# KTH-RPL/HiMo

Hardware: AMD Instinct MI355X
Metric: lidar_frames_per_sec_120k (higher is better)
Workload: dtype f16x2 (two-term split fp16, x = h + l with exact subnormals, on the matrix cores; float32 accumulate; ~22-bit products); 1 GPU; per-frame pipeline: pillarise 3 sweeps (512x512 grid) -> SeFlow++-style encoder/decoder + GRU head (random-init, self-specified: reference network source absent) -> per-point flow -> ego-motion removal + dt0 + flow2compDis -> comp_dis; points_per_frame=120000, sweeps_per_frame=3, parallelism=frames sharded x1, refined_output=False, batches_in_flight=3, matrix_arithmetic=f16x2, samples_per_backbone_launch=16, collectives=none (single process)

## Files before the change

himo_amd/csrc/conv.hip:

```cpp
#include "conv_plan.h"

namespace himo {

template <int KS, int S, int BN, int EPI, int MI>
__global__ __launch_bounds__(256) void conv_mfma_kernel(ConvArgs a) {
    constexpr int BM = 64 * MI, BK = 16, TH = 4 * MI, TW = 16;
    constexpr int PH = KS == 1 ? 1 : (TH - 1) * S + KS;
    constexpr int PW = KS == 1 ? BM : (TW - 1) * S + KS;
    constexpr int PP = PH * PW + 1;
    constexpr int WN = BN / 2, NI = WN / 32;
    constexpr int T = KS * KS;
    constexpr bool kPatchDouble = S == 1;
    constexpr int kPatchBufs = kPatchDouble ? 2 : 1;
    constexpr int kPatchItems = PH * PW * (BK / 4);
    constexpr int kPatchPerThread = (kPatchItems + 255) / 256;
    constexpr int kWPerThread = BK * (BN / 4) / 256;
    constexpr int kPatchFloats = kPatchBufs * BK * PP, kWFloats = 2 * BK * BN;
    static_assert(kPatchFloats % 4 == 0, "weight slabs stay 16-byte aligned");
    __shared__ __attribute__((aligned(16))) float smem[kPatchFloats + kWFloats < 4096 ? 4096 : kPatchFloats + kWFloats];
    auto& patchT = *reinterpret_cast<float (*)[kPatchBufs][BK * PP]>(smem);
    auto& wt = *reinterpret_cast<float (*)[2][BK * BN]>(smem + kPatchFloats);

    const int n_tiles_n = (a.Cout + BN - 1) / BN;
    int bid = xcd_block_id(blockIdx.x, gridDim.x);
// ... 261 lines not shown
    const unsigned item = blockIdx.x * 256u + threadIdx.x;
    const unsigned ox = item / cq, q = item - ox * cq;
    if (ox >= 2u * (unsigned)a.W) return;
    const int oy = (int)blockIdx.y;
    const float sy = a.ry * (float)oy, sx = a.rx * (float)ox;
    const int y0 = (int)sy, x0 = (int)sx;
    const int y1 = y0 + (y0 < a.H - 1 ? 1 : 0), x1 = x0 + (x0 < a.W - 1 ? 1 : 0);
    const float ly1 = sy - (float)y0, lx1 = sx - (float)x0;
    const float ly0 = 1.f - ly1, lx0 = 1.f - lx1;
    const float* row0 = a.x + (int64_t)y0 * a.W * a.x_pitch + q * 8;
    const float* row1 = a.x + (int64_t)y1 * a.W * a.x_pitch + q * 8;
    const unsigned c0 = (unsigned)x0 * (unsigned)a.x_pitch, c1 = (unsigned)x1 * (unsigned)a.x_pitch;
    float o[8];
#pragma unroll
    for (int part = 0; part < 2; ++part) {
        const float4 v00 = *reinterpret_cast<const float4*>(row0 + c0 + part * 4), v01 = *reinterpret_cast<const float4*>(row0 + c1 + part * 4);
        const float4 v10 = *reinterpret_cast<const float4*>(row1 + c0 + part * 4), v11 = *reinterpret_cast<const float4*>(row1 + c1 + part * 4);
        o[part * 4 + 0] = ly0 * (lx0 * v00.x + lx1 * v01.x) + ly1 * (lx0 * v10.x + lx1 * v11.x);
        o[part * 4 + 1] = ly0 * (lx0 * v00.y + lx1 * v01.y) + ly1 * (lx0 * v10.y + lx1 * v11.y);
        o[part * 4 + 2] = ly0 * (lx0 * v00.z + lx1 * v01.z) + ly1 * (lx0 * v10.z + lx1 * v11.z);
        o[part * 4 + 3] = ly0 * (lx0 * v00.w + lx1 * v01.w) + ly1 * (lx0 * v10.w + lx1 * v11.w);
    }
    unsigned h[8], l[8];
#pragma unroll
    for (int k = 0; k < 8; ++k) split2_rounded(o[k], h[k], l[k]);
    unsigned char* rec = reinterpret_cast<unsigned char*>(a.y + ((int64_t)oy * (2 * a.W) + ox) * a.y_pitch + (q >> 1) * 16) + (q & 1) * 16;
    *reinterpret_cast<uint4*>(rec) = make_uint4(h[0] | (h[1] << 16), h[2] | (h[3] << 16), h[4] | (h[5] << 16), h[6] | (h[7] << 16));
    *reinterpret_cast<uint4*>(rec + 32) = make_uint4(l[0] | (l[1] << 16), l[2] | (l[3] << 16), l[4] | (l[5] << 16), l[6] | (l[7] << 16));
}

constexpr int kUpRows = 8;
template <int CQ>
__global__ __launch_bounds__(256) void upsample2x_split_lds_kernel(UpArgs a) {
    constexpr int PX = 256 / CQ, NC = PX / 2 + 2, NR = kUpRows / 2 + 2, C = CQ * 8, C4 = C / 4;
    constexpr int CP = C + 4;
    __shared__ __attribute__((aligned(16))) float tile[NR * NC * CP];
    a.x += (int64_t)blockIdx.z * a.x_bs;
    a.y += (int64_t)blockIdx.z * a.y_bs;
    const int ox0 = (int)blockIdx.x * PX, oy0 = (int)blockIdx.y * kUpRows;
    const int cy0 = (int)(a.ry * (float)oy0), cx0 = (int)(a.rx * (float)ox0);
    for (int e = threadIdx.x; e < NR * NC * C4; e += 256) {
        const int px = e / C4, j = e - px * C4;
        const int r = px / NC, c = px - r * NC;
        const int yy = min(cy0 + r, a.H - 1), xx = min(cx0 + c, a.W - 1);
        *reinterpret_cast<float4*>(&tile[px * CP + j * 4]) = *reinterpret_cast<const float4*>(a.x + ((int64_t)yy * a.W + xx) * a.x_pitch + j * 4);
    }
    __syncthreads();
    const int q = threadIdx.x % CQ, p = threadIdx.x / CQ;
    const int ox = ox0 + p;
    if (ox >= 2 * a.W) return;
    const float sx = a.rx * (float)ox;
    const int x0 = (int)sx;
    const int x1 = x0 + (x0 < a.W - 1 ? 1 : 0);
    const float lx1 = sx - (float)x0, lx0 = 1.f - lx1;
    const int t0 = (x0 - cx0) * CP + q * 8, t1 = (x1 - cx0) * CP + q * 8;
#pragma unroll
    for (int r = 0; r < kUpRows; ++r) {
        const int oy = oy0 + r;
        if (oy >= 2 * a.H) break;
        const float sy = a.ry * (float)oy;
        const int y0 = (int)sy;
        const int y1 = y0 + (y0 < a.H - 1 ? 1 : 0);
        const float ly1 = sy - (float)y0, ly0 = 1.f - ly1;
        const float* r0 = &tile[(y0 - cy0) * NC * CP], * r1 = &tile[(y1 - cy0) * NC * CP];
        float o[8];
#pragma unroll
        for (int part = 0; part < 2; ++part) {
            const float4 v00 = *reinterpret_cast<const float4*>(r0 + t0 + part * 4), v01 = *reinterpret_cast<const float4*>(r0 + t1 + part * 4);
            const float4 v10 = *reinterpret_cast<const float4*>(r1 + t0 + part * 4), v11 = *reinterpret_cast<const float4*>(r1 + t1 + part * 4);
            o[part * 4 + 0] = ly0 * (lx0 * v00.x + lx1 * v01.x) + ly1 * (lx0 * v10.x + lx1 * v11.x);
            o[part * 4 + 1] = ly0 * (lx0 * v00.y + lx1 * v01.y) + ly1 * (lx0 * v10.y + lx1 * v11.y);
            o[part * 4 + 2] = ly0 * (lx0 * v00.z + lx1 * v01.z) + ly1 * (lx0 * v10.z + lx1 * v11.z);
            o[part * 4 + 3] = ly0 * (lx0 * v00.w + lx1 * v01.w) + ly1 * (lx0 * v10.w + lx1 * v11.w);
        }
        unsigned h[8], l[8];
#pragma unroll
        for (int k = 0; k < 8; ++k) split2_rounded(o[k], h[k], l[k]);
        unsigned char* rec = reinterpret_cast<unsigned char*>(a.y + ((int64_t)oy * (2 * a.W) + ox) * a.y_pitch + (q >> 1) * 16) + (q & 1) * 16;
        *reinterpret_cast<uint4*>(rec) = make_uint4(h[0] | (h[1] << 16), h[2] | (h[3] << 16), h[4] | (h[5] << 16), h[6] | (h[7] << 16));
        *reinterpret_cast<uint4*>(rec + 32) = make_uint4(l[0] | (l[1] << 16), l[2] | (l[3] << 16), l[4] | (l[5] << 16), l[6] | (l[7] << 16));
    }
}

template <int KS, int S, int BN, int MI>
static void launch_epi(const ConvPlan& p, hipStream_t s) {
    switch (p.epi) {
        case kEpiBias: hipLaunchKernelGGL((conv_mfma_kernel<KS, S, BN, kEpiBias, MI>), p.grid, dim3(256), 0, s, p.args); break;
        case kEpiBiasBnGelu: hipLaunchKernelGGL((conv_mfma_kernel<KS, S, BN, kEpiBiasBnGelu, MI>), p.grid, dim3(256), 0, s, p.args); break;
        case kEpiBiasGelu: hipLaunchKernelGGL((conv_mfma_kernel<KS, S, BN, kEpiBiasGelu, MI>), p.grid, dim3(256), 0, s, p.args); break;
        case kEpiGruZR: hipLaunchKernelGGL((conv_mfma_kernel<KS, S, BN, kEpiGruZR, MI>), p.grid, dim3(256), 0, s, p.args); break;
        case kEpiBiasRelu: hipLaunchKernelGGL((conv_mfma_kernel<KS, S, BN, kEpiBiasRelu, MI>), p.grid, dim3(256), 0, s, p.args); break;
        case kEpiReluMask: hipLaunchKernelGGL((conv_mfma_kernel<KS, S, BN, kEpiReluMask, MI>), p.grid, dim3(256), 0, s, p.args); break;
        default: hipLaunchKernelGGL((conv_mfma_kernel<KS, S, BN, kEpiGruQ, MI>), p.grid, dim3(256), 0, s, p.args); break;
    }
}

template <int KS, int S>
static void launch_tile(const ConvPlan& p, hipStream_t s) {
    if (p.bn == 128) { if (p.mi == 2) launch_epi<KS, S, 128, 2>(p, s); else launch_epi<KS, S, 128, 1>(p, s); }
    else { if (p.mi == 2) launch_epi<KS, S, 64, 2>(p, s); else launch_epi<KS, S, 64, 1>(p, s); }
}

void launch_conv_f32(const ConvPlan& p, hipStream_t s) {
    if (p.ks == 1) launch_tile<1, 1>(p, s);
    else if (p.stride == 1) launch_tile<3, 1>(p, s);
    else launch_tile<3, 2>(p, s);
}

}

using namespace himo;

extern "C" int himo_conv2d(const himo_conv_desc* d, void* stream) {
    if (!d) return HIMO_ERR_INVALID_ARGUMENT;
    ConvPlan p;
    const int st = plan_conv(*d, p);
    if (st != HIMO_OK) return st;
    hipStream_t s = (hipStream_t)stream;
    {
        ProfScope ps(p.prof_name, s);
        switch (p.family) {
            case kConvF32: launch_conv_f32(p, s); break;
            case kConvStaged: launch_conv_staged(p, s); break;
            case kConvFromL2: launch_conv_from_l2(p, s); break;
            case kConvPresplit3: launch_conv_presplit3(p, s); break;
            case kConvPresplit1: launch_conv_presplit1(p, s); break;
        }
    }
    HIMO_LAUNCH_CHECK(p.prof_name);
    return HIMO_OK;
}

extern "C" int himo_upsample2x(const float* d_x, int x_pitch, int h, int w, int c, float* d_y, int y_pitch, void* stream) {
    return himo_upsample2x_batch(1, d_x, 0, x_pitch, h, w, c, d_y, 0, y_pitch, stream);
}

extern "C" int himo_upsample2x_batch(int n, const float* d_x, int64_t x_batch_stride, int x_pitch, int h, int w, int c, float* d_y,
                                     int64_t y_batch_stride, int y_pitch, void* stream) {
    return himo_upsample2x_batch_ex(n, d_x, x_batch_stride, x_pitch, h, w, c, d_y, y_batch_stride, y_pitch, 0, stream);
}

extern "C" int himo_upsample2x_batch_ex(int n, const float* d_x, int64_t x_batch_stride, int x_pitch, int h, int w, int c, float* d_y,
                                        int64_t y_batch_stride, int y_pitch, int out_split, void* stream) {
    if (out_split && ((c & 15) || (y_pitch & 15) || (y_batch_stride & 15) || (reinterpret_cast<uintptr_t>(d_y) & 63))) return HIMO_ERR_INVALID_ARGUMENT;
    if (n < 1 || !d_x || !d_y || h < 1 || w < 1 || c < 4 || (c & 3) || (x_pitch & 3) || (y_pitch & 3) || (x_batch_stride & 3) ||
        (y_batch_stride & 3))
        return HIMO_ERR_INVALID_ARGUMENT;
    UpArgs a{};
    a.x = d_x; a.x_pitch = x_pitch; a.H = h; a.W = w; a.C = c; a.y = d_y; a.y_pitch = y_pitch;
    a.x_bs = x_batch_stride; a.y_bs = y_batch_stride; a.out_split = out_split ? 1 : 0;
    a.ry = h > 1 ? (float)(h - 1) / (float)(2 * h - 1) : 0.f;
    a.rx = w > 1 ? (float)(w - 1) / (float)(2 * w - 1) : 0.f;
    ProfScope ps("upsample2x_kernel", (hipStream_t)stream);
    if (out_split && (c == 64 || c == 128 || c == 256) && (2 * h + kUpRows - 1) / kUpRows <= 65535 && n <= 65535) {
        const int cq = c / 8, px = 256 / cq;
        const dim3 grid((2 * w + px - 1) / px, (2 * h + kUpRows - 1) / kUpRows, n);
        if (cq == 8) hipLaunchKernelGGL(upsample2x_split_lds_kernel<8>, grid, dim3(256), 0, (hipStream_t)stream, a);
        else if (cq == 16) hipLaunchKernelGGL(upsample2x_split_lds_kernel<16>, grid, dim3(256), 0, (hipStream_t)stream, a);
        else hipLaunchKernelGGL(upsample2x_split_lds_kernel<32>, grid, dim3(256), 0, (hipStream_t)stream, a);
        HIMO_LAUNCH_CHECK("upsample2x_split_lds_kernel");
        return HIMO_OK;
    }
    if (out_split && 2 * h <= 65535 && n <= 65535 && (int64_t)w * x_pitch < ((int64_t)1 << 31)) {
        const unsigned row_items = (unsigned)(2 * w) * (unsigned)(c / 8);
        hipLaunchKernelGGL(upsample2x_split_row_kernel, dim3((row_items + 255) / 256, 2 * h, n), dim3(256), 0, (hipStream_t)stream, a);
        HIMO_LAUNCH_CHECK("upsample2x_split_row_kernel");
        return HIMO_OK;
    }
    const int64_t total = (int64_t)(2 * h) * (2 * w) * (c / (out_split ? 8 : 4));
    const dim3 grid((unsigned)((total + 255) / 256), n);
    if (out_split) hipLaunchKernelGGL(upsample2x_kernel<true>, grid, dim3(256), 0, (hipStream_t)stream, a);
    else hipLaunchKernelGGL(upsample2x_kernel<false>, grid, dim3(256), 0, (hipStream_t)stream, a);
    HIMO_LAUNCH_CHECK("upsample2x_kernel");
    return HIMO_OK;
}
```

himo_amd/csrc/conv_plan.h:

```cpp
#pragma once
#include "conv_common.h"

namespace himo {

enum ConvFamily {
    kConvF32,
    kConvStaged,
    kConvFromL2,
    kConvPresplit3,
    kConvPresplit1
};

struct ConvPlan {
    ConvFamily family;
    ConvArgs args;
    int ks, stride, epi, fmt;
    int bn, mi, ph, nt;
    const void* w_packed;
    dim3 grid;
    const char* prof_name;
};

void launch_conv_f32(const ConvPlan& p, hipStream_t s);
void launch_conv_staged(const ConvPlan& p, hipStream_t s);
void launch_conv_from_l2(const ConvPlan& p, hipStream_t s);
void launch_conv_presplit3(const ConvPlan& p, hipStream_t s);
void launch_conv_presplit1(const ConvPlan& p, hipStream_t s);

inline int64_t blocks_for(const ConvArgs& a, int th, int tw, int bn) {
    const int64_t tiles = th ? (int64_t)((a.Ho + th - 1) / th) * ((a.Wo + tw - 1) / tw) : ((int64_t)a.Ho * a.Wo + tw - 1) / tw;
    return (int64_t)a.N * tiles * ((a.Cout + bn - 1) / bn);
}

inline bool below_2gb(int64_t pixels, int pitch) { return pixels * pitch * 4 < ((int64_t)1 << 31); }

inline const char* conv_prof_name(int ks, int stride, int fmt) {
    static const char* const names[3][4] = {
        {"conv1x1_mfma_kernel", "conv1x1_bf16x3_kernel", "conv1x1_f16x2_kernel", "conv1x1_bf16x2_kernel"},
        {"conv3x3_mfma_kernel", "conv3x3_bf16x3_kernel", "conv3x3_f16x2_kernel", "conv3x3_bf16x2_kernel"},
        {"conv3x3s2_mfma_kernel", "conv3x3s2_bf16x3_kernel", "conv3x3s2_f16x2_kernel", "conv3x3s2_bf16x2_kernel"}};
    return names[ks == 1 ? 0 : stride == 2 ? 2 : 1][fmt < 0 ? 0 : fmt == 1 ? 2 : fmt == 2 ? 3 : 1];
}

inline void plan_staged_tile(ConvPlan& p, int rows_per_mi, int tw, bool keep128, int hint) {
    const ConvArgs& a = p.args;
    auto blocks = [&](int bn, int mi) { return p.ks == 1 ? blocks_for(a, 0, 64 * mi, bn) : blocks_for(a, rows_per_mi * mi, tw, bn); };
    const bool can128 = a.Cout >= 128 && (a.Cout % 128) == 0;
    int bn = can128 ? 128 : 64, mi = 2;
    if (blocks(bn, mi) < 512) mi = 1;
    if (blocks(bn, mi) < 512 && bn == 128 && !keep128) bn = 64;
    const int hb = hint >> 4, hm = hint & 15;
    if ((hb == 64 || (hb == 128 && can128)) && (hm == 1 || hm == 2)) { bn = hb; mi = hm; }
    p.bn = bn; p.mi = mi;
    p.grid = dim3((unsigned)blocks(bn, mi));
}

inline void plan_rows_tile(ConvPlan& p, int ph, int mi, int nt) {
    p.ph = ph; p.mi = mi; p.nt = nt; p.bn = (4 / ph) * 32 * nt;
    p.grid = dim3((unsigned)(p.ks == 1 ? blocks_for(p.args, 0, mi * ph * 32, p.bn) : blocks_for(p.args, mi * ph, 32, p.bn)));
}

inline bool plan_from_l2(ConvPlan& p, int rows_hint) {
    ConvArgs& a = p.args;
    const bool vec = vec_store_ok(a);
    if (p.epi == kEpiGruZR || p.epi == kEpiGruQ) return false;
    if (p.fmt == 2 && (p.epi != kEpiBias || (a.act_flags & ~(kActAccumulate | kActStuffedIn)))) return false;
    if ((a.act_flags & kActAccumulate) && (p.fmt != 2 || !vec)) return false;
    if ((a.act_flags & kActStuffedIn) && (p.fmt != 2 || p.stride != 1)) return false;
    if (!below_2gb((int64_t)a.H * a.W, a.x_pitch)) return false;
    const bool ph_ok = p.stride == 1 && p.fmt != 0;
    const int ph_hint = (ph_ok && (rows_hint == 5 || rows_hint == 6)) ? 2 : (ph_ok && (rows_hint == 9 || rows_hint == 10)) ? 4 : 0;
    if (!ph_hint && rows_hint > 4) return false;
    const bool wide = a.Cout > 64 && ph_hint == 0;
    const int ph = ph_hint ? ph_hint : (wide ? 1 : 2);
    int mi = blocks_for(a, 4 * ph, 32, (4 / ph) * 32) >= 1024 ? 4 : 2;
    if (rows_hint == 4 || rows_hint == 2 || rows_hint == 1) mi = rows_hint;
    if (ph_hint) mi = rows_hint & 3;
    if (p.stride == 2) mi = (rows_hint == 1 || rows_hint == 2) ? rows_hint : (wide ? 2 : 1);
    p.family = kConvFromL2;
    plan_rows_tile(p, ph, mi, 1);
    p.prof_name = conv_prof_name(3, p.stride, p.fmt);
    if (vec && (!(a.act_flags & kActSplitOut) || !(a.Cout & 15))) a.act_flags |= kActVecStore;
    return true;
}

inline int plan_presplit(ConvPlan& p, int rows_hint) {
    ConvArgs& a = p.args;
    if (!below_2gb((int64_t)a.H * a.W, a.x_pitch)) return HIMO_ERR_UNSUPPORTED;
    if (a.act_flags & kActRowMask) {
        p.family = kConvPresplit3;
        p.prof_name = "conv3x3_masked_f16x2_kernel";
        plan_rows_tile(p, 4, 2, 2);
        return HIMO_OK;
    }
    const bool wide = a.Cout > 64, vec = vec_store_ok(a), pinned = rows_hint == 4 || rows_hint == 2 || rows_hint == 1;
    const int ph = wide ? 1 : 2;
    p.family = p.ks == 1 ? kConvPresplit1 : kConvPresplit3;
    p.prof_name = conv_prof_name(p.ks, p.stride, 1);
    if (vec) a.act_flags |= kActVecStore;
    if (p.ks == 1) {
        int mi = wide ? 4 : 2;
        while (mi > 1 && blocks_for(a, 0, mi * ph * 32, (4 / ph) * 32) < 2048) mi >>= 1;
        if (pinned) mi = rows_hint;
        plan_rows_tile(p, ph, !wide && mi == 4 ? 2 : mi, 1);
    } else if (p.stride == 2) {
        plan_rows_tile(p, ph, wide ? 2 : 1, 1);
    } else if (!wide && rows_hint == 8 && vec) {
        plan_rows_tile(p, 4, 2, 2);
    } else if (wide && rows_hint == 12 && vec) {
        plan_rows_tile(p, a.Cout % 256 == 0 ? 1 : 2, 4, 2);
    } else {
        int mi = blocks_for(a, 4 * ph, 32, (4 / ph) * 32) >= 1024 ? 4 : 2;
        if (pinned) mi = rows_hint;
        plan_rows_tile(p, ph, !wide && mi == 4 ? 2 : mi, 1);
    }
    return HIMO_OK;
}

inline int plan_conv(const himo_conv_desc& d, ConvPlan& p) {
    if (!d.x || !d.w || !d.y) return HIMO_ERR_INVALID_ARGUMENT;
    if (d.n < 1 || d.h < 1 || d.w_in < 1 || d.cin < 1 || d.cout < 1) return HIMO_ERR_INVALID_ARGUMENT;
    if (!(d.ksize == 1 || d.ksize == 3) || !(d.stride == 1 || d.stride == 2)) return HIMO_ERR_UNSUPPORTED;
    if (d.ksize == 1 && d.stride != 1) return HIMO_ERR_UNSUPPORTED;
    if (d.epilogue < 0 || d.epilogue > kEpiReluMask) return HIMO_ERR_INVALID_ARGUMENT;
    if (d.epilogue == kEpiBiasBnGelu && (!d.scale || !d.shift)) return HIMO_ERR_INVALID_ARGUMENT;
    const bool gru = d.epilogue == kEpiGruZR || d.epilogue == kEpiGruQ;
    if (gru && (!d.aux_in || !d.aux_out)) return HIMO_ERR_INVALID_ARGUMENT;
    if (d.epilogue == kEpiReluMask && !d.aux_in) return HIMO_ERR_INVALID_ARGUMENT;
    if ((d.cin & 3) || (d.cout & 3) || (d.x_pitch & 3) || (d.x_batch_stride & 3) || !aligned16(d.x) || !aligned16(d.w))
        return HIMO_ERR_UNSUPPORTED;
    const int n_outer = d.n_outer > 1 ? d.n_outer : 1;
    if (n_outer > 1 && ((d.x_outer_stride & 3) || (d.y_outer_stride & 3))) return HIMO_ERR_INVALID_ARGUMENT;
    p = ConvPlan{};
    p.ks = d.ksize; p.stride = d.stride; p.epi = d.epilogue; p.fmt = d.packed_format; p.w_packed = d.w_packed;
    ConvArgs& a = p.args;
    a.x = d.x; a.x_batch_stride = d.x_batch_stride; a.x_pitch = d.x_pitch;
    a.w = d.w; a.bias = d.bias; a.scale = d.scale; a.shift = d.shift;
    a.y = d.y; a.y_batch_stride = d.y_batch_stride; a.y_pitch = d.y_pitch;
    a.N = d.n * n_outer; a.n_inner = d.n; a.x_outer_stride = d.x_outer_stride; a.y_outer_stride = d.y_outer_stride;
    a.H = d.h; a.W = d.w_in; a.Cin = d.cin; a.Cout = d.cout;
    a.Ho = d.stride == 2 ? (d.h + 1) / 2 : d.h;
    a.Wo = d.stride == 2 ? (d.w_in + 1) / 2 : d.w_in;
    a.aux_in = d.aux_in; a.aux_in_pitch = d.aux_in_pitch; a.aux_out = d.aux_out; a.aux_out_pitch = d.aux_out_pitch;
    a.act_flags = d.act_layout;
    a.range_seen = (d.act_layout & kActSplitOut) ? d.d_range_seen : nullptr;

    if (d.act_layout & kActRowMask) {
        if (!d.d_mask || (reinterpret_cast<uintptr_t>(d.d_mask) & 7u)) return HIMO_ERR_INVALID_ARGUMENT;
        if (d.act_layout != (kActRowMask | kActSplitIn) || !d.w_packed || d.packed_format != 1 || d.ksize != 3 || d.stride != 1 ||
            d.cout > 64 || (d.w_in & 31) || (d.epilogue != kEpiBias && d.epilogue != kEpiBiasBnGelu) || (d.cin & 15) || (d.x_pitch & 15))
            return HIMO_ERR_UNSUPPORTED;
        a.mask = reinterpret_cast<const unsigned long long*>(d.d_mask);
        a.mask_batch_stride = d.mask_batch_stride; a.mask_outer_stride = d.mask_outer_stride;
    }
    const bool gemm_acc = d.act_layout == kActAccumulate && d.w_packed && d.ksize == 1 && d.epilogue == kEpiBias && (d.packed_format == 0 || d.packed_format == 2);
    if (d.act_layout & (kActAccumulate | kActStuffedIn)) {
        if (!gemm_acc && ((d.act_layout & ~(kActAccumulate | kActStuffedIn)) || !d.w_packed || d.packed_format != 2 || d.ksize != 3 ||
                          d.stride != 1 || d.epilogue != kEpiBias))
            return HIMO_ERR_UNSUPPORTED;
        if ((d.act_layout & kActStuffedIn) && ((d.h & 1) || (d.w_in & 1) || !below_2gb((int64_t)(d.h / 2) * (d.w_in / 2), d.x_pitch)))
            return HIMO_ERR_UNSUPPORTED;
    } else if (d.act_layout && !(d.act_layout & kActRowMask)) {
        if ((d.act_layout & ~(kActSplitIn | kActSplitOut)) || !d.w_packed || d.packed_format != 1) return HIMO_ERR_UNSUPPORTED;
        if (d.ksize == 1 && !(d.act_layout & kActSplitIn)) return HIMO_ERR_UNSUPPORTED;
        if (d.epilogue != kEpiBias && d.epilogue != kEpiBiasBnGelu) return HIMO_ERR_UNSUPPORTED;
        if (((d.act_layout & kActSplitIn) && ((d.cin & 15) || (d.x_pitch & 15))) ||
            ((d.act_layout & kActSplitOut) && ((d.cout & 15) || (d.y_pitch & 15))))
            return HIMO_ERR_UNSUPPORTED;
    }

    const int hint = d.tile_hint, rows_hint = hint & 15;
    const bool l2_hint = hint == 0 || (hint & 0x1000);
    if (!d.w_packed || (d.stride == 2 && (gru || !l2_hint))) {
        p.family = kConvF32;
        plan_staged_tile(p, 4, 16, d.epilogue == kEpiGruZR, hint);
        p.prof_name = conv_prof_name(d.ksize, d.stride, -1);
        if (d.ksize == 1 && vec_store_ok(a) && !(a.Cout & 31) && (d.epilogue != kEpiReluMask || (aligned16(a.aux_in) && !(a.aux_in_pitch & 3))))
            a.act_flags |= kActVecStore;
        return HIMO_OK;
    }
    if (a.act_flags & kActSplitIn) return plan_presplit(p, rows_hint);
    const bool gemm_accumulate = gemm_acc && (int64_t)a.Ho * a.Wo * a.y_pitch < (1ll << 30);
    const bool from_l2 = d.ksize == 3 && l2_hint;
    if (a.act_flags && !gemm_accumulate && !from_l2) return HIMO_ERR_UNSUPPORTED;
    if (from_l2 && plan_from_l2(p, rows_hint)) return HIMO_OK;
    if (d.ksize == 3 && (hint & 0x1000) && rows_hint > 4) return HIMO_ERR_UNSUPPORTED;
    if (d.stride != 1) return HIMO_ERR_UNSUPPORTED;
    if (!below_2gb((int64_t)a.H * a.W, a.x_pitch)) return HIMO_ERR_UNSUPPORTED;
    if (d.packed_format == 2 && (d.ksize != 1 || (d.epilogue != kEpiBias && d.epilogue != kEpiReluMask) || (a.act_flags && !gemm_accumulate)))
        return HIMO_ERR_UNSUPPORTED;
    p.family = kConvStaged;
    plan_staged_tile(p, 2, 32, false, hint);
    p.prof_name = conv_prof_name(d.ksize, 1, d.packed_format);
    return HIMO_OK;
}

}
```

himo_amd/csrc/convsg.hip:

```cpp
#include "conv_plan.h"
#include "bf16x3.h"
#include <type_traits>

namespace himo {

__device__ __attribute__((aligned(64))) unsigned char g_zero_page[64];


__device__ inline void glds16(const void* gsrc, unsigned lds_dst) {
    unsigned keep;
    asm volatile("s_mov_b32 %0, m0\n\ts_mov_b32 m0, %2\n\ts_nop 0\n\tglobal_load_lds_dwordx4 %1, off\n\ts_mov_b32 m0, %0"
                 : "=&s"(keep) : "v"(gsrc), "s"(lds_dst) : "memory");
}

template <int EPI, int PH, int MI, bool OSPLIT, int S, int NT = 1>
__global__ __launch_bounds__(256, NT == 2 ? (MI == 2 ? 3 : 2) : (S == 2 || MI == 4) ? 3 : 4)
void conv3_presplit_kernel(ConvArgs a, const unsigned short* __restrict__ wpk) {
    constexpr int TW = 32, TH = MI * PH, PHt = S == 1 ? TH + 2 : 2 * TH + 1, PWP = S == 1 ? 40 : 80, UPR = PWP / 16;
    constexpr int kRow = PWP * 64, kBuf = (PHt * kRow + 1023) / 1024 * 1024;
    constexpr int kUnits = S == 1 ? (PHt * PWP + 15) / 16 : PHt * UPR, kUPW = (kUnits + 3) / 4;
    constexpr int BN = (4 / PH) * 32 * NT;
    __shared__ __attribute__((aligned(1024))) unsigned char patch[2 * kBuf];

    const int n_tiles_n = (a.Cout + BN - 1) / BN;
// ... 279 lines not shown
#pragma unroll
            for (int kx = 0; kx < 3; ++kx) {
                const int p = c + kx, f = (p >> 2) & 3;
                rd[mi][kx] = r * kRow + p * 64 + ((lh ^ f) << 4);
                asm volatile("" : "+v"(rd[mi][kx]));
            }
        }
        floatx16 acc[MIW];
#pragma unroll
        for (int mi = 0; mi < MIW; ++mi)
#pragma unroll
            for (int r = 0; r < 16; ++r) acc[mi][r] = 0.f;

        uint4 bq[3][2];
        load_b(0, 0, bq[0]);
        load_b(1, 0, bq[1]);
        asm volatile("s_waitcnt vmcnt(0)" ::: "memory");
        __syncthreads();

#pragma unroll 1
        for (int slab = 0; slab < slabs; ++slab) {
            const int buf = slab & 1;
            const bool more = slab + 1 < slabs;
            const int nslab = more ? slab + 1 : slab;
            if (more) stage(slab + 1, buf ^ 1);
#pragma unroll 1
            for (int ky = 0; ky < 3; ++ky) {
                const int rowoff = buf * kBuf + ky * kRow;
#pragma unroll
                for (int kx = 0; kx < 3; ++kx) {
                    const int tap = ky * 3 + kx;
                    const int t2 = tap + 2;
                    load_b(t2 < 9 ? t2 : t2 - 9, t2 < 9 ? slab : nslab, bq[(kx + 2) % 3]);
                    f16x8 af[MIW][2];
#pragma unroll
                    for (int s = 0; s < 2; ++s)
#pragma unroll
                        for (int mi = 0; mi < MIW; ++mi)
                            af[mi][s] = *reinterpret_cast<const f16x8*>(&patch[(rd[mi][kx] ^ (s << 5)) + rowoff]);
                    const uint4 (&bcur)[2] = bq[kx];
#define HIMO_TERM16(SA, SB)                                                                                        \
    _Pragma("unroll") for (int mi = 0; mi < MIW; ++mi)                                                               \
        acc[mi] = __builtin_amdgcn_mfma_f32_32x32x16_f16(af[mi][SA], __builtin_bit_cast(f16x8, bcur[SB]), acc[mi], 0, 0, 0);
                    { HIMO_TERM16(1, 0) HIMO_TERM16(0, 1) HIMO_TERM16(0, 0) }
#undef HIMO_TERM16
                    __builtin_amdgcn_sched_group_barrier(0x020, 2, 0);
                    __builtin_amdgcn_sched_group_barrier(0x100, MIW * 2, 0);
                    __builtin_amdgcn_sched_group_barrier(0x008, MIW * 3, 0);
                }
            }
            if (more) {
                asm volatile("s_waitcnt vmcnt(4)" ::: "memory");
                __syncthreads();
            }
        }

        int ln = threadIdx.x;
        asm volatile("" : "+v"(ln));
        const int co = ct * 32 + (ln & 31), lhe = (ln >> 5) & 1;
        const int cl = co < a.Cout ? co : a.Cout - 1;
        float eA, eB;
        epi_affine<EPI>(kF16AccScale, a.bias ? a.bias[cl] : 0.f, EPI == kEpiBiasBnGelu ? a.scale[cl] : 1.f, EPI == kEpiBiasBnGelu ? a.shift[cl] : 0.f, eA, eB);
#pragma unroll
        for (int mi = 0; mi < MIW; ++mi) {
            const int e0 = (first + mi) * 32 + 4 * lhe;
#pragma unroll
            for (int g = 0; g < 4; ++g) {
                const unsigned four = *reinterpret_cast<const unsigned*>(&s_list[e0 + 8 * g]);
#pragma unroll
                for (int j = 0; j < 4; ++j) {
                    const int pxl = (four >> (8 * j)) & 255;
                    if (e0 + 8 * g + j < n_occ && co < a.Cout)
                        yout[((int64_t)(oy0 + (pxl >> 5)) * a.Wo + (ox0 + (pxl & 31))) * a.y_pitch + co] = epi_activate<EPI>(acc[mi][4 * g + j], eA, eB);
                }
            }
        }
    };
    if (mine_n == 1) { run(std::integral_constant<int, 1>{}); return; }
    if (mine_n == 2) { run(std::integral_constant<int, 2>{}); return; }
    if (mine_n == 3) { run(std::integral_constant<int, 3>{}); return; }
    run(std::integral_constant<int, 4>{});
}

template <int EPI, int PH, int MI, bool OSPLIT>
__global__ __launch_bounds__(256, 4)
void conv1_presplit_kernel(ConvArgs a, const unsigned short* __restrict__ wpk) {
    constexpr int G = 2, TH = MI * PH, BM = TH * 32;
    constexpr int kSeg = 32 * 64, kSlab = TH * kSeg, kBuf = G * kSlab;
    constexpr int kUnits = G * TH * 2, kUPW = (kUnits + 3) / 4;
    constexpr int BN = (4 / PH) * 32;
    __shared__ __attribute__((aligned(1024))) unsigned char patch[2 * kBuf < 16384 ? 16384 : 2 * kBuf];

    const int n_tiles_n = (a.Cout + BN - 1) / BN;
    int bid = xcd_block_id(blockIdx.x, gridDim.x);
    const int tn = bid % n_tiles_n; bid /= n_tiles_n;
    const int64_t rows = (int64_t)a.Ho * a.Wo;
    const int tiles = (int)((rows + BM - 1) / BM);
    const int img = bid / tiles;
    const int64_t row0 = (int64_t)(bid % tiles) * BM;
    const unsigned char* __restrict__ xin = reinterpret_cast<const unsigned char*>(a.x + image_offset(img, a.n_inner, a.x_batch_stride, a.x_outer_stride));
    const int slabs = a.Cin >> 4, steps = (slabs + G - 1) / G;

    const int wave = __builtin_amdgcn_readfirstlane(threadIdx.x >> 6), lane = threadIdx.x & 63;
    const int wp = wave % PH, wc = wave / PH;
    const int li = lane & 31, lh = lane >> 5;
    const int co = tn * BN + wc * 32 + li;
    const bool co_ok = co < a.Cout;
    const unsigned lds_base = (unsigned)(uintptr_t)(__attribute__((address_space(3))) unsigned char*)(&patch[0]);

    int src[kUPW];
#pragma unroll
    for (int k = 0; k < kUPW; ++k) {
        const int u = wave + 4 * k;
        const int g = u / (2 * TH), seg = (u >> 1) % TH, px = (u & 1) * 16 + (lane >> 2);
        const int64_t pix = row0 + seg * 32 + px;
        const int sl = (lane & 3) ^ ((px >> 2) & 3);
        src[k] = (u < kUnits && pix < rows) ? (int)(pix * a.x_pitch * 4 + sl * 16 + g * 64) : -1;
    }
    const unsigned char* zero = g_zero_page + (lane & 3) * 16;
    auto stage = [&](int step, int buf) {
#pragma unroll
        for (int k = 0; k < kUPW; ++k) {
            const int u = wave + 4 * k;
            if (u < kUnits) {
                const int g = u / (2 * TH);
                const bool ok = src[k] >= 0 && step * G + g < slabs;
                glds16(ok ? xin + (unsigned)(src[k] + step * (G * 64)) : zero, lds_base + buf * kBuf + g * kSlab + ((u >> 1) % TH) * kSeg + (u & 1) * 1024);
            }
        }
    };

    floatx16 acc[MI];
#pragma unroll
    for (int mi = 0; mi < MI; ++mi)
#pragma unroll
        for (int r = 0; r < 16; ++r) acc[mi][r] = 0.f;

    const int co_ld = co_ok ? co : a.Cout - 1;
    const unsigned char* __restrict__ wb = reinterpret_cast<const unsigned char*>(wpk);
    const unsigned b_lane = (unsigned)co_ld * 32u + (unsigned)lh * 16u, b_plane = (unsigned)a.Cout * 32u;
    auto load_b = [&](int slab, uint4 (&b)[2]) {
        const unsigned off = (unsigned)slab * (2u * b_plane) + b_lane;
        b[0] = *reinterpret_cast<const uint4*>(wb + off);
        b[1] = *reinterpret_cast<const uint4*>(wb + (off + b_plane));
    };
    int rd[2];
#pragma unroll
    for (int s = 0; s < 2; ++s) rd[s] = wp * MI * kSeg + li * 64 + (((2 * s + lh) ^ ((li >> 2) & 3)) << 4);

    uint4 bq[2][2];
    stage(0, 0);
    load_b(0, bq[0]);
    asm volatile("s_waitcnt vmcnt(0)" ::: "memory");
    __syncthreads();

#pragma unroll 1
    for (int step = 0; step < steps; ++step) {
        const int buf = step & 1;
        const bool more = step + 1 < steps;
        if (more) stage(step + 1, buf ^ 1);
#pragma unroll
        for (int g = 0; g < G; ++g) {
            const int nslab = step * G + g + 1;
            load_b(nslab < slabs ? nslab : slabs - 1, bq[(g + 1) & 1]);
            f16x8 af[MI][2];
#pragma unroll
            for (int s = 0; s < 2; ++s)
#pragma unroll
                for (int mi = 0; mi < MI; ++mi)
                    af[mi][s] = *reinterpret_cast<const f16x8*>(&patch[rd[s] + buf * kBuf + g * kSlab + mi * kSeg]);
            const uint4 (&bcur)[2] = bq[g & 1];
#define HIMO_TERM16(SA, SB)                                                                                        \
    _Pragma("unroll") for (int mi = 0; mi < MI; ++mi)                                                                \
        acc[mi] = __builtin_amdgcn_mfma_f32_32x32x16_f16(af[mi][SA], __builtin_bit_cast(f16x8, bcur[SB]), acc[mi], 0, 0, 0);
            HIMO_TERM16(1, 0) HIMO_TERM16(0, 1) HIMO_TERM16(0, 0)
#undef HIMO_TERM16
        }
        if (more) {
            asm volatile("s_waitcnt vmcnt(2)" ::: "memory");
            __syncthreads();
        }
    }

    float* __restrict__ yout = a.y + image_offset(img, a.n_inner, a.y_batch_stride, a.y_outer_stride);
    float eA, eB;
    epi_affine<EPI>(kF16AccScale, a.bias ? a.bias[co_ld] : 0.f, EPI == kEpiBiasBnGelu ? a.scale[co_ld] : 1.f, EPI == kEpiBiasBnGelu ? a.shift[co_ld] : 0.f, eA, eB);
    if (a.act_flags & kActVecStore) {
        __syncthreads();
        unsigned char* stg = patch + wave * 4096;
#pragma unroll
        for (int mi = 0; mi < MI; ++mi) {
            const int64_t pix0 = row0 + (wp * MI + mi) * 32;
            const int64_t left = rows - pix0;
            unsigned word[16];
#pragma unroll
            for (int r = 0; r < 16; ++r) {
                const float v = epi_activate<EPI>(acc[mi][r], eA, eB);
                word[r] = OSPLIT ? split_word(v, li & 1) : __builtin_bit_cast(unsigned, v);
                if (OSPLIT && mi == 0 && r == 0) note_range(a, (4 * lh < left && tn * BN + wc * 32 + li < a.Cout) ? v : 0.f);
            }
            store_block_vec<OSPLIT>(a, yout, stg, word, lane, pix0, left < 0 ? 0 : left > 32 ? 32 : (int)left, tn * BN + wc * 32);
        }
        return;
    }
    if (!co_ok) return;
#pragma unroll
    for (int mi = 0; mi < MI; ++mi) {
#pragma unroll
        for (int r = 0; r < 16; ++r) {
            const int64_t pix = row0 + (wp * MI + mi) * 32 + (r & 3) + 8 * (r >> 2) + 4 * lh;
            if (pix < rows) {
                const float v = epi_activate<EPI>(acc[mi][r], eA, eB);
                if (OSPLIT) split_store<kEpiBias, true>(a, yout, pix, co, v, 1.f, 0.f);
                else yout[pix * a.y_pitch + co] = v;
            }
        }
    }
}

#define HIMO_SG(KERNEL, E, O, ...) hipLaunchKernelGGL((KERNEL<E, PH, MI, O, ##__VA_ARGS__>), p.grid, dim3(256), 0, s, p.args, (const unsigned short*)p.w_packed)
#define HIMO_SG_EPI(KERNEL, ...)                                                                                                          \
    do {                                                                                                                                  \
        const bool osplit = (p.args.act_flags & kActSplitOut) != 0;                                                                       \
        if (p.epi == kEpiBias) { if (osplit) HIMO_SG(KERNEL, kEpiBias, true, ##__VA_ARGS__); else HIMO_SG(KERNEL, kEpiBias, false, ##__VA_ARGS__); } \
        else { if (osplit) HIMO_SG(KERNEL, kEpiBiasBnGelu, true, ##__VA_ARGS__); else HIMO_SG(KERNEL, kEpiBiasBnGelu, false, ##__VA_ARGS__); }       \
    } while (0)

template <int PH, int MI>
static void launch_sg1(const ConvPlan& p, hipStream_t s) { HIMO_SG_EPI(conv1_presplit_kernel); }

template <int PH, int MI, int S = 1, int NT = 1>
static void launch_sg(const ConvPlan& p, hipStream_t s) { HIMO_SG_EPI(conv3_presplit_kernel, S, NT); }
#undef HIMO_SG_EPI
#undef HIMO_SG

void launch_conv_presplit1(const ConvPlan& p, hipStream_t s) {
    if (p.ph == 1) {
        if (p.mi == 4) launch_sg1<1, 4>(p, s);
        else if (p.mi == 2) launch_sg1<1, 2>(p, s);
        else launch_sg1<1, 1>(p, s);
    } else {
        if (p.mi == 2) launch_sg1<2, 2>(p, s);
        else launch_sg1<2, 1>(p, s);
    }
}

void launch_conv_presplit3(const ConvPlan& p, hipStream_t s) {
    if (p.args.act_flags & kActRowMask) {
        if (p.epi == kEpiBias) hipLaunchKernelGGL((conv3_rowmask_kernel<kEpiBias>), p.grid, dim3(256), 0, s, p.args, (const unsigned short*)p.w_packed);
        else hipLaunchKernelGGL((conv3_rowmask_kernel<kEpiBiasBnGelu>), p.grid, dim3(256), 0, s, p.args, (const unsigned short*)p.w_packed);
        return;
    }
    if (p.stride == 2) { if (p.ph == 1) launch_sg<1, 2, 2>(p, s); else launch_sg<2, 1, 2>(p, s); }
    else if (p.nt == 2) {
        if (p.ph == 4) launch_sg<4, 2, 1, 2>(p, s);
        else if (p.ph == 1) launch_sg<1, 4, 1, 2>(p, s);
        else launch_sg<2, 4, 1, 2>(p, s);
    }
    else if (p.ph == 1) {
        if (p.mi == 4) launch_sg<1, 4>(p, s);
        else if (p.mi == 2) launch_sg<1, 2>(p, s);
        else launch_sg<1, 1>(p, s);
    } else {
        if (p.mi == 2) launch_sg<2, 2>(p, s);
        else launch_sg<2, 1>(p, s);
    }
}

}
```

himo_amd/seflow/model.py:

```python
from __future__ import annotations

import ctypes

import numpy as np
import torch

from .. import _lib
from . import spec

EPI_BIAS, EPI_BIAS_BN_GELU, EPI_BIAS_GELU, EPI_GRU_ZR, EPI_GRU_Q = range(5)


class ConvDesc(ctypes.Structure):
    _fields_ = [("x", ctypes.c_void_p), ("x_batch_stride", ctypes.c_int64), ("x_pitch", ctypes.c_int),
                ("w", ctypes.c_void_p), ("bias", ctypes.c_void_p), ("scale", ctypes.c_void_p), ("shift", ctypes.c_void_p),
                ("y", ctypes.c_void_p), ("y_batch_stride", ctypes.c_int64), ("y_pitch", ctypes.c_int),
                ("n", ctypes.c_int), ("h", ctypes.c_int), ("w_in", ctypes.c_int), ("cin", ctypes.c_int),
                ("cout", ctypes.c_int), ("ksize", ctypes.c_int), ("stride", ctypes.c_int), ("epilogue", ctypes.c_int),
                ("aux_in", ctypes.c_void_p), ("aux_in_pitch", ctypes.c_int),
                ("aux_out", ctypes.c_void_p), ("aux_out_pitch", ctypes.c_int), ("w_packed", ctypes.c_void_p),
                ("tile_hint", ctypes.c_int), ("packed_format", ctypes.c_int),
                ("n_outer", ctypes.c_int), ("x_outer_stride", ctypes.c_int64), ("y_outer_stride", ctypes.c_int64),
                ("act_layout", ctypes.c_int), ("range_seen", ctypes.c_void_p),
                ("mask", ctypes.c_void_p), ("mask_batch_stride", ctypes.c_int64), ("mask_outer_stride", ctypes.c_int64)]
# ... 270 lines not shown
            self._sparse_dec4 = on
            self.drop_plan()

    @property
    def B0(self):
        return self._B0

    @B0.setter
    def B0(self, buf):
        self._B0 = buf
        self.drop_plan()
        self.reset_images()

    MAX_RANGE_SLOTS = 63

    def clear_nonfinite(self):
        _lib.check(self.lib.himo_clear_u32(self.guard.data_ptr(), self.guard.numel(), _lib.stream_handle()), "himo_clear_u32")

    def _range_word(self, wname: str) -> int:
        k = self._range_slots.setdefault(wname, len(self._range_slots))
        if k >= self.MAX_RANGE_SLOTS:
            raise RuntimeError("more split-output layers than guard words")
        return self.guard.data_ptr() + 4 * (1 + k)

    def guard_verdict(self, words) -> str | None:
        w = [int(v) for v in words]
        if w[0] != 0:
            return "overflow"
        if w[-1] != 0 and any(w[1 + k] == 0 for k in self._range_slots.values()):
            return "underflow"
        return None

    def reset_images(self):
        for st in getattr(self, "_pt", ()):
            for ws in st["ws_slots"]:
                _lib.check(self.lib.himo_pillar_occupancy_reset(ws.data_ptr(), ws.numel(), self.W, self.H, _lib.stream_handle()),
                           "himo_pillar_occupancy_reset")

    def _use_sample(self, i: int):
        st = self._pt[i]
        self._sample = i
        self.ws_slots, self.xyz_t, self.pid, self.offsets = st["ws_slots"], st["xyz_t"], st["pid"], st["offsets"]

    def _conv(self, x, x_bs, x_pitch, wname, y, y_bs, y_pitch, n, h, w, cin, cout, ks, stride, epi, x_off=0, y_off=0,
              scale=None, shift=None, aux_in=None, aux_in_pitch=0, aux_out=None, aux_out_pitch=0, bias=None, batched=True,
              act=0, mask=None):
        d = ConvDesc()
        d.x = x.data_ptr() + 4 * x_off; d.x_batch_stride = x_bs; d.x_pitch = x_pitch
        if batched and self._nb > 1:
            d.n_outer, d.x_outer_stride, d.y_outer_stride = self._nb, x.stride(0), y.stride(0)
        d.w = self.p[f"{wname}.weight"].data_ptr()
        d.bias = (self.p[f"{wname}.bias"] if bias is None else bias).data_ptr()
        d.scale = None if scale is None else scale.data_ptr()
        d.shift = None if shift is None else shift.data_ptr()
        d.y = y.data_ptr() + 4 * y_off; d.y_batch_stride = y_bs; d.y_pitch = y_pitch
        d.n, d.h, d.w_in, d.cin, d.cout, d.ksize, d.stride, d.epilogue = n, h, w, cin, cout, ks, stride, epi
        d.aux_in = None if aux_in is None else aux_in.data_ptr(); d.aux_in_pitch = aux_in_pitch
        d.aux_out = None if aux_out is None else aux_out.data_ptr(); d.aux_out_pitch = aux_out_pitch
        pk = self.packed.get(f"{wname}.weight")
        d.w_packed = None if pk is None else pk.data_ptr()
        d.packed_format = self.packed_format
        d.act_layout = act if self.split_acts else 0
        if mask is not None:
            d.act_layout |= ACT_ROW_MASK
            d.mask, d.mask_batch_stride, d.mask_outer_stride = mask.data_ptr(), 0, mask.stride(0)
        if (d.act_layout & ACT_SPLIT_OUT) and self.packed_format == 1 and epi in (EPI_BIAS, EPI_BIAS_BN_GELU):
            d.range_seen = self._range_word(wname)
        key = (n * max(d.n_outer, 1), h, w, cin, cout, ks, stride, epi, pk is not None, d.act_layout)
        if self.autotune and key not in self.tiles:
            self.tiles[key] = self._tune(d)
        d.tile_hint = self.tiles.get(key, 0)
        if self._recording is not None and epi not in (EPI_GRU_ZR, EPI_GRU_Q):
            op = HimoOp(); op.kind = 0; op.conv = d
            self._recording.append(op)
        _lib.check(self.lib.himo_conv2d(ctypes.byref(d), _lib.stream_handle()), f"himo_conv2d({wname})")

    def _tune(self, d: "ConvDesc") -> int:
        if d.epilogue in (EPI_GRU_ZR, EPI_GRU_Q) or (d.act_layout & ACT_ROW_MASK):
            return 0
        cands = [(bn << 4) | mi for bn in (128, 64) if not (bn == 128 and d.cout % 128) for mi in (2, 1)]
        if d.act_layout:
            if d.stride == 2 and (d.act_layout & ACT_SPLIT_IN):
                return 0
            cands = [0x1000 | 4, 0x1000 | 2, 0x1000 | 1] if d.ksize == 1 else []
        if d.w_packed and d.ksize == 3:
            cands += [0x1000 | 4, 0x1000 | 2, 0x1000 | 1] if d.stride == 1 else [0x1000 | 2, 0x1000 | 1]
            if d.stride == 1 and (d.act_layout & ACT_SPLIT_IN) and self.packed_format == 1:
                cands.append(0x1000 | (8 if d.cout <= 64 else 12))
        if len(cands) < 2:
            return cands[0] if cands else 0
        return fastest_tile_hint(self.lib, d, cands, warmup=2)

    def _up(self, x, x_pitch, h, w, c, y, y_pitch, out_split=False):
        nb = self._nb
        osp = 1 if (out_split and self.split_acts) else 0
        if self._recording is not None:
            op = HimoOp(); op.kind = 1
            op.up_x, op.up_x_pitch, op.up_h, op.up_w, op.up_c, op.up_y, op.up_y_pitch = x.data_ptr(), x_pitch, h, w, c, y.data_ptr(), y_pitch
            op.up_n, op.up_x_batch_stride, op.up_y_batch_stride = nb, x.stride(0), y.stride(0)
            op.up_out_split = osp
            self._recording.append(op)
        _lib.check(self.lib.himo_upsample2x_batch_ex(nb, x.data_ptr(), x.stride(0) if nb > 1 else 0, x_pitch, h, w, c, y.data_ptr(),
                                                     y.stride(0) if nb > 1 else 0, y_pitch, osp, _lib.stream_handle()), "himo_upsample2x_batch_ex")

    def backbone(self, n_samples: int = 1):
        if not 1 <= n_samples <= self.max_batch:
            raise ValueError(f"n_samples must be in 1..{self.max_batch}")
        self._nb = n_samples
        if self.packed_format == 1:
            self._ran_word.fill_(1)
        plan = self._plans.get(n_samples)
        if self.use_plan and plan is not None:
            ops, n = plan
            _lib.check(self.lib.himo_run_ops(ctypes.addressof(ops), n, 1 if self.use_graph else 0, _lib.stream_handle()), "himo_run_ops")
            return self.DEC
        self._recording = [] if self.use_plan else None
        self.encoder()
        self.decoder()
        if self._recording is not None:
            rec, self._recording = self._recording, None
            self._plans[n_samples] = ((HimoOp * len(rec))(*rec), len(rec))
        return self.DEC

    def __del__(self):
        try:
            self.drop_plan()
        except Exception:
            pass

    def drop_plan(self):
        for plan in self._plans.values():
            self.lib.himo_ops_release(ctypes.addressof(plan[0]))
        self._plans = {}

    def encoder(self):
        H, W, F = self.H, self.W, self.F
        p = self.p
        stages = [("enc1", 4, 32, 64, H, W, self.E1, self.F1), ("enc2", 6, 64, 128, H // 2, W // 2, self.E2, self.F2),
                  ("enc3", 6, 128, 256, H // 4, W // 4, self.E3, self.F3)]
        src, src_bs, src_pitch = self.B0, 32, 32 * F
        for stage, n_conv, cin, cout, h, w, pingpong, catbuf in stages:
            ho, wo = h // 2, w // 2
            for i in range(n_conv):
                name = f"{stage}.{i}"
                last = i == n_conv - 1
                dst = catbuf if last else pingpong[i % 2]
                dst_bs, dst_pitch = (cout, cout * F) if last else (ho * wo * cout, cout)
                act = ACT_SPLIT_IN | ACT_SPLIT_OUT
                if i == 0:
                    self._conv(src, src_bs, src_pitch, name, dst, dst_bs, dst_pitch, F, h, w, cin, cout, 3, 2,
                               EPI_BIAS_BN_GELU, scale=p[f"{name}.scale"], shift=p[f"{name}.shift"], act=act)
                else:
                    self._conv(src, src_bs, src_pitch, name, dst, dst_bs, dst_pitch, F, ho, wo, cout, cout, 3, 1,
                               EPI_BIAS_BN_GELU, scale=p[f"{name}.scale"], shift=p[f"{name}.shift"], act=act)
                src, src_bs, src_pitch = dst, dst_bs, dst_pitch

    def decoder(self):
        H, W, F = self.H, self.W, self.F
        IN, IO = ACT_SPLIT_IN, ACT_SPLIT_IN | ACT_SPLIT_OUT
        fold = self.fold_decoder
        def block(name, coarse, c_in, ch, cw, tmp, cat, skip, skip_c, lat, out, work, nxt=None):
            if coarse is not None:
                self._conv(coarse, 0, c_in, f"{name}.u1", tmp, 0, lat, 1, 1, ch * cw, c_in, lat, 1, 1, EPI_BIAS, act=IN)
            self._up(tmp, lat, ch, cw, lat, cat, 2 * lat, out_split=True)
            self._conv(skip, 0, skip_c, f"{name}.u3", cat, 0, 2 * lat, 1, 1, 4 * ch * cw, skip_c, lat, 1, 1, EPI_BIAS, y_off=lat, act=IO)
            self._conv(cat, 0, 2 * lat, f"{name}.u4", work[0], 0, out, 1, 2 * ch, 2 * cw, 2 * lat, out, 3, 1, EPI_BIAS, act=IO)
            if fold and nxt is not None:
# ... 222 lines not shown
```

Baseline: 776.4 frames/s.

## Add row-sum upsample kernel and prefetch-ahead weight pipeline for 1x1 presplit conv

```diff
diff --git a/himo_amd/csrc/conv.hip b/himo_amd/csrc/conv.hip
--- a/himo_amd/csrc/conv.hip
+++ b/himo_amd/csrc/conv.hip
@@ -367,6 +367,68 @@
     }
 }
 
+template <int CQ, int ROWS>
+__global__ __launch_bounds__(256) void upsample2x_split_rowsum_kernel(UpArgs a) {
+    constexpr int PX = 256 / CQ, NC = PX / 2 + 2, NR = ROWS / 2 + 2, C = CQ * 8, C4 = C / 4;
+    constexpr int CP = C + 4;
+    __shared__ __attribute__((aligned(16))) float tile[NR * NC * CP];
+    a.x += (int64_t)blockIdx.z * a.x_bs;
+    a.y += (int64_t)blockIdx.z * a.y_bs;
+    const int ox0 = (int)blockIdx.x * PX, oy0 = (int)blockIdx.y * ROWS;
+    const int cy0 = (int)(a.ry * (float)oy0), cx0 = (int)(a.rx * (float)ox0);
+    for (int e = threadIdx.x; e < NR * NC * C4; e += 256) {
+        const int px = e / C4, j = e - px * C4;
+        const int r = px / NC, c = px - r * NC;
+        const int yy = min(cy0 + r, a.H - 1), xx = min(cx0 + c, a.W - 1);
+        *reinterpret_cast<float4*>(&tile[px * CP + j * 4]) = *reinterpret_cast<const float4*>(a.x + ((int64_t)yy * a.W + xx) * a.x_pitch + j * 4);
+    }
+    __syncthreads();
+    const int q = threadIdx.x % CQ, p = threadIdx.x / CQ;
+    const int ox = ox0 + p;
+    if (ox >= 2 * a.W) return;
+    const float sx = a.rx * (float)ox;
+    const int x0 = (int)sx;
+    const int x1 = x0 + (x0 < a.W - 1 ? 1 : 0);
+    const float lx1 = sx - (float)x0, lx0 = 1.f - lx1;
+    const int t0 = (x0 - cx0) * CP + q * 8, t1 = (x1 - cx0) * CP + q * 8;
+    auto rowsum = [&](int tr, float (&s)[8]) {
+        const float* rp = &tile[tr * NC * CP];
+#pragma unroll
+        for (int part = 0; part < 2; ++part) {
+            const float4 v0 = *reinterpret_cast<const float4*>(rp + t0 + part * 4), v1 = *reinterpret_cast<const float4*>(rp + t1 + part * 4);
+            s[part * 4 + 0] = lx0 * v0.x + lx1 * v1.x;
+            s[part * 4 + 1] = lx0 * v0.y + lx1 * v1.y;
+            s[part * 4 + 2] = lx0 * v0.z + lx1 * v1.z;
+            s[part * 4 + 3] = lx0 * v0.w + lx1 * v1.w;
+        }
+    };
+    const int n_rows = min(ROWS, 2 * a.H - oy0);
+    int r = 0;
+    auto rows_of = [&](int t, const float (&up)[8], float (&dn)[8]) {
+        rowsum(t + 1, dn);
+        for (; r < n_rows; ++r) {
+            const int oy = oy0 + r;
+            const float sy = a.ry * (float)oy;
+            const int y0 = (int)sy;
+            if (y0 - cy0 != t) break;
+            const float ly1 = sy - (float)y0, ly0 = 1.f - ly1;
+            unsigned h[8], l[8];
+#pragma unroll
+            for (int k = 0; k < 8; ++k) split2_rounded(ly0 * up[k] + ly1 * dn[k], h[k], l[k]);
+            unsigned char* rec = reinterpret_cast<unsigned char*>(a.y + ((int64_t)oy * (2 * a.W) + ox) * a.y_pitch + (q >> 1) * 16) + (q & 1) * 16;
+            *reinterpret_cast<uint4*>(rec) = make_uint4(h[0] | (h[1] << 16), h[2] | (h[3] << 16), h[4] | (h[5] << 16), h[6] | (h[7] << 16));
+            *reinterpret_cast<uint4*>(rec + 32) = make_uint4(l[0] | (l[1] << 16), l[2] | (l[3] << 16), l[4] | (l[5] << 16), l[6] | (l[7] << 16));
+        }
+    };
+    float s0[8], s1[8];
+    rowsum(0, s0);
+#pragma unroll 1
+    for (int t = 0; t < NR - 1 && r < n_rows; t += 2) {
+        rows_of(t, s0, s1);
+        if (t + 1 < NR - 1 && r < n_rows) rows_of(t + 1, s1, s0);
+    }
+}
+
 template <int KS, int S, int BN, int MI>
 static void launch_epi(const ConvPlan& p, hipStream_t s) {
     switch (p.epi) {
@@ -437,12 +499,20 @@
     a.ry = h > 1 ? (float)(h - 1) / (float)(2 * h - 1) : 0.f;
     a.rx = w > 1 ? (float)(w - 1) / (float)(2 * w - 1) : 0.f;
     ProfScope ps("upsample2x_kernel", (hipStream_t)stream);
-    if (out_split && (c == 64 || c == 128 || c == 256) && (2 * h + kUpRows - 1) / kUpRows <= 65535 && n <= 65535) {
+    const int pinned = out_split >> 4, up_rows = pinned == 1 || pinned == 2 ? kUpRows : pinned == 3 ? 4 : c == 256 ? kUpRows : 4;
+    if (out_split && (c == 64 || c == 128 || c == 256) && (2 * h + up_rows - 1) / up_rows <= 65535 && n <= 65535) {
         const int cq = c / 8, px = 256 / cq;
-        const dim3 grid((2 * w + px - 1) / px, (2 * h + kUpRows - 1) / kUpRows, n);
-        if (cq == 8) hipLaunchKernelGGL(upsample2x_split_lds_kernel<8>, grid, dim3(256), 0, (hipStream_t)stream, a);
-        else if (cq == 16) hipLaunchKernelGGL(upsample2x_split_lds_kernel<16>, grid, dim3(256), 0, (hipStream_t)stream, a);
-        else hipLaunchKernelGGL(upsample2x_split_lds_kernel<32>, grid, dim3(256), 0, (hipStream_t)stream, a);
+        const dim3 grid((2 * w + px - 1) / px, (2 * h + up_rows - 1) / up_rows, n);
+#define HIMO_UP(KERNEL, ...)                                                                                            \
+    do {                                                                                                                \
+        if (cq == 8) hipLaunchKernelGGL((KERNEL<8, ##__VA_ARGS__>), grid, dim3(256), 0, (hipStream_t)stream, a);        \
+        else if (cq == 16) hipLaunchKernelGGL((KERNEL<16, ##__VA_ARGS__>), grid, dim3(256), 0, (hipStream_t)stream, a); \
+        else hipLaunchKernelGGL((KERNEL<32, ##__VA_ARGS__>), grid, dim3(256), 0, (hipStream_t)stream, a);               \
+    } while (0)
+        if (pinned == 1) HIMO_UP(upsample2x_split_lds_kernel);
+        else if (up_rows == 4) HIMO_UP(upsample2x_split_rowsum_kernel, 4);
+        else HIMO_UP(upsample2x_split_rowsum_kernel, kUpRows);
+#undef HIMO_UP
         HIMO_LAUNCH_CHECK("upsample2x_split_lds_kernel");
         return HIMO_OK;
     }
diff --git a/himo_amd/csrc/conv_plan.h b/himo_amd/csrc/conv_plan.h
--- a/himo_amd/csrc/conv_plan.h
+++ b/himo_amd/csrc/conv_plan.h
@@ -16,6 +16,7 @@
     ConvArgs args;
     int ks, stride, epi, fmt;
     int bn, mi, ph, nt;
+    bool ahead;
     const void* w_packed;
     dim3 grid;
     const char* prof_name;
@@ -84,7 +85,7 @@
     return true;
 }
 
-inline int plan_presplit(ConvPlan& p, int rows_hint) {
+inline int plan_presplit(ConvPlan& p, int rows_hint, bool ahead_hint) {
     ConvArgs& a = p.args;
     if (!below_2gb((int64_t)a.H * a.W, a.x_pitch)) return HIMO_ERR_UNSUPPORTED;
     if (a.act_flags & kActRowMask) {
@@ -103,6 +104,7 @@
         while (mi > 1 && blocks_for(a, 0, mi * ph * 32, (4 / ph) * 32) < 2048) mi >>= 1;
         if (pinned) mi = rows_hint;
         plan_rows_tile(p, ph, !wide && mi == 4 ? 2 : mi, 1);
+        p.ahead = pinned && ahead_hint && p.mi <= 2;
     } else if (p.stride == 2) {
         plan_rows_tile(p, ph, wide ? 2 : 1, 1);
     } else if (!wide && rows_hint == 8 && vec) {
@@ -179,7 +181,7 @@
             a.act_flags |= kActVecStore;
         return HIMO_OK;
     }
-    if (a.act_flags & kActSplitIn) return plan_presplit(p, rows_hint);
+    if (a.act_flags & kActSplitIn) return plan_presplit(p, rows_hint, (hint & 0x10) != 0);
     const bool gemm_accumulate = gemm_acc && (int64_t)a.Ho * a.Wo * a.y_pitch < (1ll << 30);
     const bool from_l2 = d.ksize == 3 && l2_hint;
     if (a.act_flags && !gemm_accumulate && !from_l2) return HIMO_ERR_UNSUPPORTED;
diff --git a/himo_amd/csrc/convsg.hip b/himo_amd/csrc/convsg.hip
--- a/himo_amd/csrc/convsg.hip
+++ b/himo_amd/csrc/convsg.hip
@@ -385,7 +385,7 @@
     run(std::integral_constant<int, 4>{});
 }
 
-template <int EPI, int PH, int MI, bool OSPLIT>
+template <int EPI, int PH, int MI, bool OSPLIT, bool AHEAD = false>
 __global__ __launch_bounds__(256, 4)
 void conv1_presplit_kernel(ConvArgs a, const unsigned short* __restrict__ wpk) {
     constexpr int G = 2, TH = MI * PH, BM = TH * 32;
@@ -451,39 +451,83 @@
 #pragma unroll
     for (int s = 0; s < 2; ++s) rd[s] = wp * MI * kSeg + li * 64 + (((2 * s + lh) ^ ((li >> 2) & 3)) << 4);
 
-    uint4 bq[2][2];
-    stage(0, 0);
-    load_b(0, bq[0]);
-    asm volatile("s_waitcnt vmcnt(0)" ::: "memory");
-    __syncthreads();
-
-#pragma unroll 1
-    for (int step = 0; step < steps; ++step) {
-        const int buf = step & 1;
-        const bool more = step + 1 < steps;
-        if (more) stage(step + 1, buf ^ 1);
-#pragma unroll
-        for (int g = 0; g < G; ++g) {
-            const int nslab = step * G + g + 1;
-            load_b(nslab < slabs ? nslab : slabs - 1, bq[(g + 1) & 1]);
-            f16x8 af[MI][2];
-#pragma unroll
-            for (int s = 0; s < 2; ++s)
-#pragma unroll
-                for (int mi = 0; mi < MI; ++mi)
-                    af[mi][s] = *reinterpret_cast<const f16x8*>(&patch[rd[s] + buf * kBuf + g * kSlab + mi * kSeg]);
-            const uint4 (&bcur)[2] = bq[g & 1];
 #define HIMO_TERM16(SA, SB)                                                                                        \
     _Pragma("unroll") for (int mi = 0; mi < MI; ++mi)                                                                \
         acc[mi] = __builtin_amdgcn_mfma_f32_32x32x16_f16(af[mi][SA], __builtin_bit_cast(f16x8, bcur[SB]), acc[mi], 0, 0, 0);
-            HIMO_TERM16(1, 0) HIMO_TERM16(0, 1) HIMO_TERM16(0, 0)
+    if constexpr (AHEAD) {
+        auto settle = [](uint4 (&b)[2]) {
+            asm volatile("" : "+v"(b[0].x), "+v"(b[0].y), "+v"(b[0].z), "+v"(b[0].w), "+v"(b[1].x), "+v"(b[1].y), "+v"(b[1].z), "+v"(b[1].w));
+        };
+        uint4 bc[G][2], bn[G][2];
+        stage(0, 0);
+#pragma unroll
+        for (int g = 0; g < G; ++g) load_b(g < slabs ? g : slabs - 1, bc[g]);
+        asm volatile("s_waitcnt vmcnt(0)" ::: "memory");
+#pragma unroll
+        for (int g = 0; g < G; ++g) settle(bc[g]);
+        __syncthreads();
+#pragma unroll 1
+        for (int step = 0; step < steps; ++step) {
+            const int buf = step & 1;
+            const bool more = step + 1 < steps;
+            if (more) {
+#pragma unroll
+                for (int g = 0; g < G; ++g) {
+                    const int nslab = (step + 1) * G + g;
+                    load_b(nslab < slabs ? nslab : slabs - 1, bn[g]);
+                }
+                stage(step + 1, buf ^ 1);
+            }
+#pragma unroll
+            for (int g = 0; g < G; ++g) {
+                f16x8 af[MI][2];
+#pragma unroll
+                for (int s = 0; s < 2; ++s)
+#pragma unroll
+                    for (int mi = 0; mi < MI; ++mi)
+                        af[mi][s] = *reinterpret_cast<const f16x8*>(&patch[rd[s] + buf * kBuf + g * kSlab + mi * kSeg]);
+                const uint4 (&bcur)[2] = bc[g];
+                HIMO_TERM16(1, 0) HIMO_TERM16(0, 1) HIMO_TERM16(0, 0)
+            }
+            if (more) {
+                asm volatile("s_waitcnt vmcnt(0)" ::: "memory");
+#pragma unroll
+                for (int g = 0; g < G; ++g) { settle(bn[g]); bc[g][0] = bn[g][0]; bc[g][1] = bn[g][1]; }
+                __syncthreads();
+            }
+        }
+    } else {
+        uint4 bq[2][2];
+        stage(0, 0);
+        load_b(0, bq[0]);
+        asm volatile("s_waitcnt vmcnt(0)" ::: "memory");
+        __syncthreads();
+
+#pragma unroll 1
+        for (int step = 0; step < steps; ++step) {
+            const int buf = step & 1;
+            const bool more = step + 1 < steps;
+            if (more) stage(step + 1, buf ^ 1);
+#pragma unroll
+            for (int g = 0; g < G; ++g) {
+                const int nslab = step * G + g + 1;
+                load_b(nslab < slabs ? nslab : slabs - 1, bq[(g + 1) & 1]);
+                f16x8 af[MI][2];
+#pragma unroll
+                for (int s = 0; s < 2; ++s)
+#pragma unroll
+                    for (int mi = 0; mi < MI; ++mi)
+                        af[mi][s] = *reinterpret_cast<const f16x8*>(&patch[rd[s] + buf * kBuf + g * kSlab + mi * kSeg]);
+                const uint4 (&bcur)[2] = bq[g & 1];
+                HIMO_TERM16(1, 0) HIMO_TERM16(0, 1) HIMO_TERM16(0, 0)
+            }
+            if (more) {
+                asm volatile("s_waitcnt vmcnt(2)" ::: "memory");
+                __syncthreads();
+            }
+        }
+    }
 #undef HIMO_TERM16
-        }
-        if (more) {
-            asm volatile("s_waitcnt vmcnt(2)" ::: "memory");
-            __syncthreads();
-        }
-    }
 
     float* __restrict__ yout = a.y + image_offset(img, a.n_inner, a.y_batch_stride, a.y_outer_stride);
     float eA, eB;
@@ -530,7 +574,12 @@
     } while (0)
 
 template <int PH, int MI>
-static void launch_sg1(const ConvPlan& p, hipStream_t s) { HIMO_SG_EPI(conv1_presplit_kernel); }
+static void launch_sg1(const ConvPlan& p, hipStream_t s) {
+    if constexpr (MI <= 2) {
+        if (p.ahead) { HIMO_SG_EPI(conv1_presplit_kernel, true); return; }
+    }
+    HIMO_SG_EPI(conv1_presplit_kernel);
+}
 
 template <int PH, int MI, int S = 1, int NT = 1>
 static void launch_sg(const ConvPlan& p, hipStream_t s) { HIMO_SG_EPI(conv3_presplit_kernel, S, NT); }
diff --git a/himo_amd/seflow/model.py b/himo_amd/seflow/model.py
--- a/himo_amd/seflow/model.py
+++ b/himo_amd/seflow/model.py
@@ -376,7 +376,7 @@
         if d.act_layout:
             if d.stride == 2 and (d.act_layout & ACT_SPLIT_IN):
                 return 0
-            cands = [0x1000 | 4, 0x1000 | 2, 0x1000 | 1] if d.ksize == 1 else []
+            cands = [0x1000 | 4, 0x1000 | 2, 0x1000 | 1, 0x1010 | 2, 0x1010 | 1] if d.ksize == 1 else []
         if d.w_packed and d.ksize == 3:
             cands += [0x1000 | 4, 0x1000 | 2, 0x1000 | 1] if d.stride == 1 else [0x1000 | 2, 0x1000 | 1]
             if d.stride == 1 and (d.act_layout & ACT_SPLIT_IN) and self.packed_format == 1:
```

Result: no change. 778.6 frames/s (median of 6 runs) (+0.3%).
